# grigoriy-chirkov/primesim

Measured on AMD Instinct MI355X. Metric: simulated memory accesses/sec (uncore) at 1024 cores; % HBM roofline, higher is better.
Workload: dtype int64

## Files before the change

primesim_amd/csrc/engine.hip:

```cpp

#ifndef __HIPCC_RTC__
#include <hip/hip_runtime.h>
#include <stdint.h>
#endif

#if defined(__HIPCC_RTC__) || defined(PU_JIT_OFFLINE)
#include "primeuncore.h"
#else
#include "../../include/primeuncore.h"
#endif
#include "geometry.h"

namespace {

#ifdef PU_JIT_GEO
#include PU_JIT_GEO
#endif

template <bool LH, int NL, class T>
__device__ __forceinline__ T off_v(T c) {
#ifdef PU_JIT_GEO
    if constexpr (!LH && NL == 1) {
        uint32_t lo, hi;
        asm("s_mov_b32 %0, %1" : "=s"(lo) : "s"((uint32_t)(uint64_t)c));
// ... 665 lines not shown
        x = (int)(rem - yq * w);
        y = (int)yq;
        z = (int)zq;
    } else {
        const uint32_t yq = div_magic((uint32_t)id, c.w_magic);
        x = (int)((uint32_t)id - yq * w);
        y = (int)yq;
        z = 0;
    }
}
__device__ __forceinline__ int net_route_link(const NetCtx& c, int h, int sx, int sy, int sz, int rx, int ry, int rz,
                                              int hx, int hy) {
    const int w = c.w, w1 = c.w - 1;
    const bool e = rx > sx, n = ry > sy, u = rz > sz;
    const bool inx = h < hx, iny = h < hx + hy;
    const int hy_ = h - hx, hz_ = h - hx - hy;
    const int ax = e ? sx + h : sx - h - 1;
    const int ay = n ? sy + hy_ : sy - hy_ - 1;
    if (c.net_type != 1) return inx ? sy * w1 + ax : (w + rx) * w1 + ay;
    const int az = u ? sz + hz_ : sz - hz_ - 1;
    const int blk = w * w * w1;
    return inx ? (sz * w + sy) * w1 + ax : iny ? blk + (sz * w + rx) * w1 + ay : 2 * blk + (ry * w + rx) * w1 + az;
}


template <bool LH>
__device__ __forceinline__ void ring_dma(const NetCtx& c, int q, uint32_t head, uint32_t cnt, int slot) {
    const int ln = lane_id();
    const AS1 v2u64* R = q_ring(c, q);
    const uint32_t last = cnt - 1;
    const AS1 v2u64* ga = R + ((head + __builtin_elementwise_min((uint32_t)ln, last)) & (PU_QRING - 1));
    const AS1 v2u64* gb = R + ((head + __builtin_elementwise_min((uint32_t)ln + 64, last)) & (PU_QRING - 1));
    const uint32_t la = (uint32_t)(uintptr_t)(__attribute__((address_space(3))) v2u64*)ring_slot<LH>(slot);
    const uint32_t lo = __builtin_amdgcn_readfirstlane(la), hi = lo + 64 * sizeof(v2u64);
    unsigned keep;
    asm volatile(
        "s_waitcnt lgkmcnt(0)\n\t"
        "s_mov_b32 %0, m0\n\t"
        "s_mov_b32 m0, %3\n\t"
        "s_nop 0\n\t"
        "global_load_lds_dwordx4 %1, off\n\t"
        "s_mov_b32 m0, %4\n\t"
        "s_nop 0\n\t"
        "global_load_lds_dwordx4 %2, off\n\t"
        "s_mov_b32 m0, %0"
        : "=&s"(keep)
        : "v"(ga), "v"(gb), "s"(lo), "s"(hi)
        : "memory");
}
template <bool LH>
__device__ __forceinline__ void ring_from_lds(int slot, RingView& v) {
    const int ln = lane_id();
    const v2u64* r = ring_slot<LH>(slot);
    const v2u64 a = r[ln], b = r[ln + 64];
    v = RingView{a.x, a.y, b.x, b.y};
}

template <bool X4>
__device__ __forceinline__ void lds_dma(const AS1 char* src, uint32_t lds_base) {
    const uint32_t lo = __builtin_amdgcn_readfirstlane(lds_base);
    unsigned keep;
    if (X4)
        asm volatile("s_waitcnt lgkmcnt(0)\n\ts_mov_b32 %0, m0\n\ts_mov_b32 m0, %2\n\ts_nop 0\n\t"
                     "global_load_lds_dwordx4 %1, off\n\ts_mov_b32 m0, %0"
                     : "=&s"(keep) : "v"(src), "s"(lo) : "memory");
    else
        asm volatile("s_waitcnt lgkmcnt(0)\n\ts_mov_b32 %0, m0\n\ts_mov_b32 m0, %2\n\ts_nop 0\n\t"
                     "global_load_lds_dword %1, off\n\ts_mov_b32 m0, %0"
                     : "=&s"(keep) : "v"(src), "s"(lo) : "memory");
}
template <class T>
__device__ __forceinline__ uint32_t lds_addr(T* p) {
    return (uint32_t)(uintptr_t)(__attribute__((address_space(3))) T*)p;
}

static __shared__ v4u32 lds_dir_a[32];
static __shared__ uint32_t lds_dir_w[2][32];

#ifndef PU_PAIR_WINDOW
#define PU_PAIR_WINDOW 1
#endif
template <bool LH, bool WIDE>
constexpr bool pair_window() { return PU_PAIR_WINDOW && !LH && !WIDE; }
template <bool LH, int NL, bool WIDE>
__device__ __forceinline__ uint64_t net_transmit(const Geo* __restrict__ g, char* base_in, int src, int dst, int len,
                                                 uint64_t timer, uint32_t& hq_head, bool& pair, int len2,
                                                 int64_t base_t, int tpre) {
    constexpr bool PW = pair_window<LH, WIDE>();
    PROF_T(p_pre);
    NetCtx c;
    AS1 char* base = (AS1 char*)(char*)uni64((uint64_t)base_in);
    c.qhdr = base + OFF(g->off_qhdr);
    c.qring = base + OFF(g->off_qring);
    c.hdr_c = (uint32_t)g->nqueues * PU_HDR_AB;
    c.p0 = (uint32_t)g->header_flits;
    c.p1 = (uint32_t)g->plen_blk;
    c.router = (uint32_t)g->router_delay;
    c.link_delay = (uint32_t)g->link_delay;
    c.inject = (uint32_t)g->inject_delay;
    c.header_flits = g->header_flits;
    c.data_width = g->data_width;
    c.w = g->net_width;
    c.net_type = g->net_type;
    c.w_magic = (uint32_t)g->w_magic;
    c.w2_magic = (uint32_t)g->w2_magic;
    c.w2 = g->w2;
    c.blk_len = g->blk_len;
    c.plen_blk = g->plen_blk;
    src = (int)uni32((uint32_t)src);
    dst = (int)uni32((uint32_t)dst);
    len = (int)uni32((uint32_t)len);
    timer = uni64(timer);
    if (src == dst) {
        pair = false;
        return 0;
    }
    const int ln = lane_id();
    int plen;
    uint64_t err = 0;
    if constexpr (WIDE) {
        plen = len == 0 ? c.header_flits
             : len == c.blk_len ? c.plen_blk
             : c.header_flits + (int)ceil((double)len / (double)c.data_width);
    } else {
        plen = len == 0 ? c.header_flits : c.plen_blk;
        if (len != 0 && len != c.blk_len) err |= PU_ERRF_QUEUE;
    }
    int sx, sy, sz, rx, ry, rz;
    net_coords(c, src, sx, sy, sz);
    net_coords(c, dst, rx, ry, rz);
    const int hx = abs(rx - sx), hy = abs(ry - sy), hz = abs(rz - sz);
    const int hops = hx + hy + hz;
    bool pw = false;
    if constexpr (PW) {
        pw = pair && 2 * hops <= 64 && (hx != 0) + (hy != 0) + (hz != 0) >= 2;
        len2 = (int)uni32((uint32_t)len2);
        if (pw && len2 != 0 && len2 != c.blk_len) err |= PU_ERRF_QUEUE;
    }
    pair = pw;
    const auto plen2 = [&]() { return len2 == 0 ? c.header_flits : c.plen_blk; };
    const int thops = pw ? 2 * hops : hops;
    uint64_t t = timer + c.inject;
    uint64_t mg1 = 0;
    PROF_ADD(PF_NPRE, p_pre);
    for (int b0 = 0; b0 < thops; b0 += 64) {
        PROF_T(p_setup);
        PROF_CNT(PF_WINDOWS, 1);
        const int h = b0 + ln;
        const int nh = thops - b0 < 64 ? thops - b0 : 64;
        int rq;
        if (PW && pw) {
            const int hh = h < thops ? h : thops - 1;
            const bool bk = hh >= hops;
            rq = net_route_link(c, bk ? hh - hops : hh, bk ? rx : sx, bk ? ry : sy, bk ? rz : sz, bk ? sx : rx,
                                bk ? sy : ry, bk ? sz : rz, hx, hy);
        } else {
            rq = net_route_link(c, h < hops ? h : hops - 1, sx, sy, sz, rx, ry, rz, hx, hy);
        }
        v4u32 ha, hb, hc;
        hdr_load<LH, WIDE>(c, rq, ha, hb, hc);
        uint64_t vcache = PU_MG1_CACHE_NONE;
        if constexpr (LH) vcache = lds_qcache[rq];
        const QState hs = hdr_state<WIDE>(c, ha, hb, hc, err);
        uint32_t vhead = hs.head, vcnt = hs.count;
        uint64_t vf0 = hs.f0;
        const uint64_t vfront = vf0;
        uint64_t vd = 0;
        [[maybe_unused]] bool need = ln < nh;
        if constexpr (LH) {
            const uint64_t wmask = (1ull << PU_MG1_WAIT_BITS) - 1;
            const bool hit = need && (vcache & wmask) != wmask && hs.n < 4294967296.0 &&
                             ((uint32_t)(vcache >> PU_MG1_WAIT_BITS) ^ (uint32_t)vcache) == (uint32_t)hs.n;
            if (hit) vd = vcache & wmask;
            need = need && !hit;
            if (ballot(need)) {
                PROF_T(p_mg1);
                const uint64_t w = mg1_wait(hs);
                if (need) vd = w;
                PROF_ADD(PF_MG1RUN, p_mg1);
            }
        } else {
            PROF_T(p_mg1);
            vd = mg1_wait(hs);
            PROF_ADD(PF_MG1RUN, p_mg1);
        }
        PROF_CNT(PF_MG1LANES, (uint64_t)nh);
        PROF_CNT(PF_MG1HITS, (uint64_t)__builtin_popcountll(ballot(ln < nh && !need)));
        PROF_CNT(PF_MG1PRESENT, (uint64_t)__builtin_popcountll(ballot(ln < nh && vcache != PU_MG1_CACHE_NONE)));
        uint64_t vfin = 0;
        uint64_t X = 0;
        const int nleg = PW && pw ? 2 : 1;
#pragma clang loop unroll(disable)
        for (int leg = 0; leg < nleg; leg++) {
        const int l0 = PW && leg ? hops : 0, l1 = PW && pw ? l0 + hops : nh;
        const int pl = PW && leg ? plen2() : plen;
        const uint64_t nhm = (l1 >= 64 ? ~0ull : ((1ull << l1) - 1)) & (~0ull << l0);
        const uint64_t lb = t + (uint64_t)(ln - l0 + 1) * c.router + (uint64_t)(ln - l0) * c.link_delay;
        const uint64_t M = ballot(vfront <= lb + (uint64_t)pl) & nhm;
        uint64_t mi = M, mc = M;
        int issued = 0, consumed = 0;
        constexpr int RPF = ring_pf<LH>();
        while (mi && issued < RPF) {
            const int jj = (int)__builtin_ctzll(mi);
            mi &= mi - 1;
            ring_dma<LH>(c, (int)rl32((uint32_t)rq, jj), rl32(vhead, jj), rl32(vcnt, jj), issued % RPF);
            issued++;
        }
        PROF_ADD(PF_NSETUP, p_setup);
        PROF_T(p_hops);
        uint64_t sh = 0;
        uint64_t t0 = t;
        if (!PW || leg == 0) {
            const uint64_t e = vd + c.link_delay + c.router;
            const uint64_t S = ballot(e >= (1ull << 26)) == 0 ? (uint64_t)scan_incl_u32((uint32_t)e) : scan_incl_u64(e);
            X = S - e;
        } else {
            t0 -= rl64(X, hops);
        }
        int js = l0;
        {
            int islot = issued % RPF, cslot = 0;
            while (js < l1) {
                const uint64_t live = nhm & (~0ull << js);
                const uint64_t A = X + (t0 + c.router + sh);
                const uint64_t cand = ballot(vfront <= A + (uint64_t)pl) & live;
                const int jt = cand ? (int)__builtin_ctzll(cand) : l1;
                const uint64_t fm = jt >= 64 ? live : live & ((1ull << jt) - 1);
                vfin = selm64(fm, vfin, A + vd + (uint64_t)pl);
                mg1 += (uint64_t)(jt - js);
                if (jt == l1) {
                    t = t0 + rl64(X, l1 - 1) + rl64(vd, l1 - 1) + c.link_delay + c.router + sh;
                    break;
                }
                PROF_T(p_tree);
                PROF_CNT(PF_TREEHOPS, 1);
                PROF_T(p_pick);
                const uint64_t tj = rl64(A, jt);
                const int q = (int)rl32((uint32_t)rq, jt);
                uint32_t head = rl32(vhead, jt), cnt = rl32(vcnt, jt);
                uint64_t f0n, f1n, d;
                RingView v;
                const bool staged = mc && jt == (int)__builtin_ctzll(mc);
                int tslot = -1;
                if (staged) {
                    mc &= mc - 1;
                    PROF_T(p_wait);
                    const int newer = issued - consumed - 1;
                    static_assert(RPF <= 3, "the three-way wait covers at most 2 newer staged rings");
                    if (newer <= 0) asm volatile("s_waitcnt vmcnt(0)" ::: "memory");
                    else if (newer == 1) asm volatile("s_waitcnt vmcnt(2)" ::: "memory");
                    else asm volatile("s_waitcnt vmcnt(4)" ::: "memory");
                    PROF_ADD(PF_NWAIT, p_wait);
                    ring_from_lds<LH>(cslot, v);
                    tslot = cslot;
                    cslot = cslot == RPF - 1 ? 0 : cslot + 1;
                    consumed++;
                } else {
                    PROF_CNT(PF_DEMAND, 1);
                    ring_load(c, q, head, cnt, v);
                }
#ifdef PU_PROF
                asm volatile("s_waitcnt lgkmcnt(0)" ::: "memory");
#endif
                PROF_ADD(PF_T_LDS, p_pick);
                d = tree_op<LH>(c, q, v, head, cnt, tj, (uint64_t)pl, c.link_delay, err, f0n, f1n, tslot);
                PROF_T(p_upd);
                if (cnt >= PU_QMAX) {
                    head = (head + 1) & (PU_QRING - 1);
                    cnt--;
                    f0n = f1n;
                }
                if (staged && mi) {
                    PROF_T(p_r);
                    const int jj = (int)__builtin_ctzll(mi);
                    mi &= mi - 1;
                    ring_dma<LH>(c, (int)rl32((uint32_t)rq, jj), rl32(vhead, jj), rl32(vcnt, jj), islot);
                    islot = islot == RPF - 1 ? 0 : islot + 1;
                    issued++;
                    PROF_ADD(PF_T_REFILL, p_r);
                }
                sh += d - rl64(vd, jt);
                wl_hop(vhead, head, vcnt, cnt, vf0, f0n, vfin, tj + d + (uint64_t)pl, jt);
                t = tj + d + c.link_delay;
                js = jt + 1;
                PROF_ADD(PF_T_UPD, p_upd);
                PROF_ADD(PF_NTREE, p_tree);
            }
        }
        if (PW && pw && leg == 0) {
            t += c.router;
            t += (uint64_t)(plen - 1);
            const uint64_t dfwd = t - timer;
            const uint64_t start = (uint64_t)(base_t + (tpre + (int)dfwd));
            timer = start - dfwd;
            t = start + c.inject;
        }
        PROF_ADD(PF_NHOPS, p_hops);
        }
        PROF_T(p_wb);
        if (ln < nh) {
            QState st = hs;
            st.head = vhead;
            st.count = vcnt;
            st.f0 = vf0;
            if constexpr (WIDE) {
                st.sum_sq = st.sum_sq + (double)plen * (double)plen;
                st.sum = st.sum + (double)plen;
                st.n = st.n + 1.0;
            } else {
                st.n = st.n + 1.0;
                if ((PW && pw && ln >= hops ? plen2() : plen) != (int)c.p0) st.sum1 = st.sum1 + 1.0;
            }
            st.newest = vfin > st.newest ? vfin : st.newest;
            q_store_hdr<LH, WIDE>(c, rq, st, vhead != hs.head || vcnt != hs.count || vf0 != hs.f0);
            if constexpr (LH) lds_hq[(hq_head + (uint32_t)ln) & (PU_HQ - 1)] = (uint16_t)rq;
        }
        if constexpr (LH) {
            hq_head += (uint32_t)nh;
            asm volatile("" ::: "memory");
            if (ln == 0) *(volatile AS3 uint32_t*)&lds_hq_head = hq_head;
        }
        PROF_ADD(PF_NWB, p_wb);
    }
    PROF_T(p_post);
    t += c.router;
    t += (uint64_t)((PW && pw ? plen2() : plen) - 1);
    const uint64_t dist = (uint64_t)thops;
    {
        const uint32_t plsum = (uint32_t)(PW && pw ? plen + plen2() : plen);
        const uint64_t tot = t - timer, fl = (uint64_t)hops * (uint64_t)plsum;
        uint32_t lo = 0, hi = 0;
        lo = wlane<SN_ACC>(lo, PW && pw ? 2u : 1u);
        lo = wlane<SN_DIST>(lo, (uint32_t)dist);
        lo = wlane<SN_TOTAL>(lo, (uint32_t)tot);
        hi = wlane<SN_TOTAL>(hi, (uint32_t)(tot >> 32));
        lo = wlane<SN_PLEN>(lo, plsum);
        lo = wlane<SN_FLITS>(lo, (uint32_t)fl);
        if (WIDE || (c.p0 | c.p1) >= (1u << 23)) hi = wlane<SN_FLITS>(hi, (uint32_t)(fl >> 32));
        lo = wlane<SN_MG1>(lo, (uint32_t)mg1);
        lds_add_u64_lanes(lds_u32addr(&lds_stat[0]) + 8u * (uint32_t)ln, ((uint64_t)hi << 32) | lo, SN_NET_LANES);
    }
    if (ballot(err != 0)) err_or(PU_ERRF_QUEUE);
    PROF_ADD(PF_NPOST, p_post);
    return t - timer;
}

#ifndef PU_PF_AHEAD
#define PU_PF_AHEAD 4
#endif
static __shared__ uint32_t lds_pf_junk[64];
__device__ __forceinline__ void pf_requests(const Geo* __restrict__ g, const char* base, const pu_req* reqs,
                                            uint64_t first, uint32_t n) {
    const int ln = lane_id();
    const uint32_t j = (uint32_t)ln >> 3, k = (uint32_t)ln & 7u;
    const bool mine = j < n;
    uint64_t addr = 0;
    int core = 0;
    if (mine) {
        const pu_req q = reqs[first + j];
        addr = q.addr;
        core = q.core;
    }
    const char* p = nullptr;
    if (mine && (uint32_t)core < (uint32_t)g->num_cores) {
        const LevelGeo& L = g->lv[0];
        const uint64_t set = set_index(addr, L.offbits, L.nsets);
        const uint64_t line0 = ((uint64_t)(uint32_t)core * L.nsets + set) * L.nways;
        if (k == 0) p = (const char*)(reqs + first + j);
        else if (k <= 2) {
            if ((k - 1) * 64 < L.nways * sizeof(LineMeta)) p = base + L.off_meta + line0 * sizeof(LineMeta) + (k - 1) * 64;
        } else if (k == 3) p = base + L.off_ts + line0 * 8;
        else if (g->sys_type == 0 && k <= 6 && (k - 4) * 64 < g->dir.nways * sizeof(DirLine)) {
            const DirGeo& D = g->dir;
            int hb = (int)((addr >> g->home_offbits) & (((uint64_t)1 << g->home_mask_bits) - 1));
            if (hb >= g->N) hb &= (1 << (g->home_mask_bits - 1)) - 1;
            const uint64_t ds = set_index(addr, D.offbits, D.nsets);
            const uint64_t dl0 = ((uint64_t)(uint32_t)hb * D.csets + (ds >> D.cset_shift)) * D.nways;
            p = base + D.off_line + dl0 * sizeof(DirLine) + (k - 4) * 64;
        }
    }
    if (p) lds_dma<false>((const AS1 char*)p, lds_addr(&lds_pf_junk[0]));
}

__device__ void mg1_helper(const Geo* __restrict__ g, const char* base, const pu_req* reqs, uint64_t b, uint64_t end) {
    const bool pf_on = !g->tlb_enable;
    uint64_t pf = b;

    const int ln = lane_id();
    uint32_t tail = 0;
    for (;;) {
        const uint32_t head = uni32(*(volatile AS3 uint32_t*)&lds_hq_head);
        if (head == tail) {
            if (uni32(*(volatile AS3 uint32_t*)&lds_main_done)) {
                if (uni32(*(volatile AS3 uint32_t*)&lds_hq_head) == tail) break;
                continue;
            }
            if (pf_on) {
                const uint64_t cur = uni64(*(volatile AS3 uint64_t*)&lds_ctl.cur);
                if (cur >= b && cur < end) {
                    const uint64_t lim = end - cur > PU_PF_AHEAD ? cur + 1 + PU_PF_AHEAD : end;
                    if (pf <= cur) pf = cur + 1;
                    if (pf < lim) {
                        pf_requests(g, base, reqs, pf, (uint32_t)(lim - pf));
                        pf = lim;
                        continue;
                    }
                }
            }
            __builtin_amdgcn_s_sleep(1);
            continue;
        }
        if (head - tail > PU_HQ) tail = head - PU_HQ;
        const uint32_t n = head - tail < 64u ? head - tail : 64u;
        if ((uint32_t)ln < n) {
            const uint32_t q = lds_hq[(tail + (uint32_t)ln) & (PU_HQ - 1)];
            volatile AS3 v4u32* H = (volatile AS3 v4u32*)&lds_qhdr[(size_t)q * PU_LDS_SLOT];
            const v4u32 a = H[0];
            asm volatile("" ::: "memory");
            const v4u32 b = H[1];
            asm volatile("" ::: "memory");
            const v4u32 a2 = H[0];
            NetCtx hc;
            hc.p0 = (uint32_t)g->header_flits;
            hc.p1 = (uint32_t)g->plen_blk;
            uint64_t herr = 0;
            const QState st = hdr_state<false>(hc, a, b, v4u32{0u, 0u, 0u, 0u}, herr);
            const uint64_t w = mg1_wait(st);
            const uint64_t wmask = (1ull << PU_MG1_WAIT_BITS) - 1;
            const bool same = a.x == a2.x && a.y == a2.y && a.z == a2.z && a.w == a2.w;
            const bool st_ok = same && !herr && w < wmask && st.n < 4294967296.0;
            if (st_ok)
                *(volatile AS3 uint64_t*)&lds_qcache[q] = w | ((uint64_t)((uint32_t)st.n ^ (uint32_t)w) << PU_MG1_WAIT_BITS);
#ifdef PU_PROF
            const uint64_t nst = __builtin_popcountll(ballot(st_ok));
            if (ln == 0) atomicAdd(&lds_prof[PF_MG1STORED], (unsigned long long)nst);
#endif
        }
        PROF_CNT(PF_MG1BATCH, 1);
        tail += n;
    }
}

template <int NL, bool LH = false, bool WIDE = false>
struct Engine {
    const Geo* __restrict__ g;
    char* base;
    int ln;

    int dly;
    bool hit;
    uint32_t hq_head;

    __device__ __forceinline__ void init_shared(int32_t pool_top, uint64_t page_next, uint64_t last_addr) const {
        lds_eng.pool_top = pool_top;
        lds_eng.stop = 0;
        lds_eng.page_next = page_next;
        lds_eng.last_addr = last_addr;
    }


    template <class T>
    __device__ __forceinline__ T* at(uint64_t off) const {
        return reinterpret_cast<T*>(base + off);
    }

    __device__ __forceinline__ NetCtx net_ctx() const {
        NetCtx c;
        c.qhdr = (AS1 char*)base + OFF(g->off_qhdr);
        c.qring = (AS1 char*)base + OFF(g->off_qring);
        c.hdr_c = (uint32_t)g->nqueues * PU_HDR_AB;
        c.p0 = c.p1 = (uint32_t)g->bus_latency;
        c.router = (uint32_t)g->router_delay;
        c.link_delay = (uint32_t)g->link_delay;
        c.inject = (uint32_t)g->inject_delay;
        c.header_flits = g->header_flits;
        c.data_width = g->data_width;
        c.w = g->net_width;
        c.net_type = g->net_type;
        return c;
    }
    __device__ __forceinline__ uint64_t transmit(int src, int dst, int len, uint64_t timer) {
        PROF_T(p0);
        bool pair = false;
        uint64_t d = net_transmit<LH, NL, WIDE>(g, base, src, dst, len, timer, hq_head, pair, 0, 0, 0);
        PROF_ADD(PF_NET, p0);
        return d;
    }
    __device__ __forceinline__ uint64_t transmit_leg(int src, int dst, int len, uint64_t timer, bool& pair, int len2,
                                                     int64_t base_t, int tpre) {
        PROF_T(p0);
        uint64_t d = net_transmit<LH, NL, WIDE>(g, base, src, dst, len, timer, hq_head, pair, len2, base_t, tpre);
        PROF_ADD(PF_NET, p0);
        return d;
    }

    __device__ __forceinline__ void set_load(SetView& v, const LineMeta* meta, const int64_t* ts,
                                             uint64_t nsets, uint64_t nways, int offbits, int idxbits,
                                             uint64_t cache_index, uint64_t addr) const {
        v.set = set_index(addr, offbits, nsets);
        v.tag = addr >> (offbits + idxbits);
        v.line0 = (uint64_t)(((uint32_t)cache_index * (uint32_t)nsets + (uint32_t)v.set) * (uint32_t)nways);
        set_chunk(v, meta, ts, nways, 0);
    }
    __device__ __forceinline__ void set_chunk(SetView& v, const LineMeta* meta, const int64_t* ts, uint64_t nways,
                                              uint32_t w0) const {
        v.w0 = w0;
        const uint64_t w = (uint64_t)w0 + (uint64_t)ln;
        if (w < nways) {
            LineMeta m = meta[v.line0 + w];
            v.mtag = m.tag;
            v.mid = m.id;
            v.mst = m.state;
            v.mts = ts[v.line0 + w];
        } else {
            v.mtag = 0;
            v.mid = 0;
            v.mst = ST_I;
            v.mts = INT64_MAX;
        }
    }
    static __device__ __forceinline__ bool wide(uint64_t nways) { return nways > 64; }
    static __device__ __forceinline__ int wl(const SetView& v, int way) { return way - (int)v.w0; }
    __device__ __forceinline__ int set_find(SetView& v, const LineMeta* meta, const int64_t* ts, uint64_t nways,
                                            int prog) const {
        if (!wide(nways)) {
            uint64_t m = ballot((uint64_t)ln < nways && v.mst != ST_I && v.mid == prog && v.mtag == v.tag);
            return m ? (int)__builtin_ctzll(m) : -1;
        }
        for (uint32_t c = 0;; c += 64) {
            if (c != v.w0) set_chunk(v, meta, ts, nways, c);
            const uint64_t m =
                ballot((uint64_t)c + (uint64_t)ln < nways && v.mst != ST_I && v.mid == prog && v.mtag == v.tag);
            if (m) return (int)c + (int)__builtin_ctzll(m);
            if ((uint64_t)c + 64 >= nways) return -1;
        }
    }
    __device__ __forceinline__ int set_replace(SetView& v, LineMeta* meta, const int64_t* ts, uint64_t nways,
                                               int offbits, int idxbits, int prog, uint32_t* old_state,
                                               uint64_t* old_addr, int* old_prog) const {
        int way = -1;
        bool invalid = false;
        if (!wide(nways)) {
            const uint64_t inv = ballot((uint64_t)ln < nways && v.mst == ST_I);
            if (inv) {
                invalid = true;
                way = (int)__builtin_ctzll(inv);
            } else {
                way = lru_way(v.mts, (uint64_t)ln < nways ? lane_here(ln) : 64, nways);
            }
        } else {
            int64_t best = INT64_MAX;
            for (uint32_t c = 0; (uint64_t)c < nways && !invalid; c += 64) {
                if (c != v.w0) set_chunk(v, meta, ts, nways, c);
                const bool mine = (uint64_t)c + (uint64_t)ln < nways;
                const uint64_t inv = ballot(mine && v.mst == ST_I);
                if (inv) {
                    invalid = true;
                    way = (int)c + (int)__builtin_ctzll(inv);
                } else {
                    const int lw = lru_way(v.mts, mine ? ln : 64, 64);
                    const int64_t t = (int64_t)rl64((uint64_t)v.mts, lw);
                    if (way < 0 || t < best) {
                        best = t;
                        way = (int)c + lw;
                    }
                }
            }
            if ((uint32_t)way - v.w0 >= 64u) set_chunk(v, meta, ts, nways, (uint32_t)way & ~63u);
        }
        const int wlane = wl(v, way);
        if (invalid) {
            *old_state = ST_I;
            *old_addr = 0;
            *old_prog = 0;
        } else {
            *old_state = rl32(v.mst, wlane);
            *old_addr = (v.set << offbits) | (rl64(v.mtag, wlane) << (offbits + idxbits));
            *old_prog = (int)rl32((uint32_t)v.mid, wlane);
        }
        if (ln == wlane) {
            v.mtag = v.tag;
            v.mid = prog;
            meta[v.line0 + (uint64_t)way] = LineMeta{v.tag, prog, v.mst};
        }
        return way;
    }
    __device__ __forceinline__ void set_state(SetView& v, LineMeta* meta, int way, uint32_t st) const {
        if (ln == wl(v, way)) {
            v.mst = st;
            meta[v.line0 + (uint64_t)way].state = st;
        }
    }
    __device__ __forceinline__ void set_ts(SetView& v, int64_t* ts, int way, int64_t t) const {
        if (ln == wl(v, way)) {
            v.mts = t;
            ts[v.line0 + (uint64_t)way] = t;
        }
    }

    __device__ __forceinline__ void mark_alive(int l, int cid) const {
        for (int k = l; k < NL; k++) {
            if constexpr (kAliveLds) {
                const uint32_t bit = (uint32_t)(alive_base(k) + cid), m = 1u << (bit & 31);
                const uint32_t w = uni32(lds_alive[bit >> 5]);
                if (!(w & m)) {
                    if (ln == (cid & 63)) at<uint32_t>(OFF(g->lv[k].off_alive))[cid] = 1u;
                    if (ln == 0) lds_alive[bit >> 5] = w | m;
                }
            } else {
                if (ln == (cid & 63)) at<uint32_t>(OFF(g->lv[k].off_alive))[cid] = 1u;
            }
            if (k + 1 < NL) cid = cid * g->lv[k].share / g->lv[k + 1].share;
        }
    }
    template <int K>
    __device__ __forceinline__ void count(uint64_t off_cnt, int cid, int which) const {
        if constexpr (kCntSum) stat_add(SN_CNT0 + 4 * K + which, 1);
        else gatomic_add_u64_lane0(at<uint64_t>(off_cnt) + (size_t)cid * 4 + which, 1ull);
    }

    __device__ __forceinline__ int dram(uint64_t addr, int64_t t) {
        stat_add(SN_DRAM, 1);
        if (g->dram_banks == 0) return g->dram_access_time;
        const uint64_t row = uni64(addr) >> g->dram_row_shift;
        const uint64_t bank = row & (uint64_t)(g->dram_banks - 1);
        const uint64_t page = (row >> g->dram_bank_shift) + 1;
        t = (int64_t)uni64((uint64_t)t);
        DramBank* B = at<DramBank>(OFF(g->off_dram)) + bank;
        const int64_t ready = (int64_t)uni64((uint64_t)B->ready);
        const uint64_t open = uni64(B->open);
        const int64_t start = ready > t ? ready : t;
// ... 161 lines not shown
        sh = idx;
    }

    enum ProbeMode { PR_NONE, PR_ONE, PR_INLINE, PR_POOL, PR_ALL };
    __device__ __forceinline__ int probe(int mode, int one, uint32_t nsh, uint64_t sh, bool inval, int reply_len, int home,
                         const Req& r, int64_t timer, int delay) {
        constexpr int last = NL - 1;
        const bool single = mode == PR_ONE;
        const int64_t base_t = single ? timer : timer + delay;
        int pipe = single ? delay : 0, mx = 0;
        int pbase = 0;
        uint64_t rem = mode == PR_POOL ? pool_word(sh) : 0ull;
        uint32_t k = 0;
        while (true) {
            int p;
            if (mode == PR_ONE) {
                if (k) break;
                p = one;
            } else if (mode == PR_INLINE) {
                if (k >= nsh) break;
                p = (int)((sh >> (16 * k)) & 0xFFFF);
            } else if (mode == PR_POOL) {
                uint64_t m = ballot(rem != 0);
                while (!m && pbase + 64 < g->dir.nwords) {
                    pbase += 64;
                    rem = pool_word(sh, pbase);
                    m = ballot(rem != 0);
                }
                if (!m) break;
                const int w = (int)__builtin_ctzll(m);
                p = (pbase + w) * 64 + (int)__builtin_ctzll(rl64(rem, w));
                if (ln == w) rem &= rem - 1;
            } else if (mode == PR_ALL) {
                if ((int)k >= g->num_cores) break;
                p = (int)k;
            } else {
                break;
            }
            k++;
            int t = pipe;
            if constexpr (pair_window<LH, WIDE>()) {
                const uint64_t start = (uint64_t)(base_t + t);
                t += inval ? down<last, true>(p, r) : down<last, false>(p, r);
#pragma clang loop unroll(disable)
                for (int back = 0; back < 2; back++) {
                    bool paired = !back;
                    t += (int)transmit_leg(back ? p : home, back ? home : p, back ? reply_len : 0,
                                           back ? (uint64_t)(base_t + t) : start, paired, reply_len, base_t, t);
                    if (paired) break;
                }
            } else {
#pragma clang loop unroll(disable)
                for (int back = 0; back < 2; back++) {
                    t += (int)transmit(back ? p : home, back ? home : p, back ? reply_len : 0, (uint64_t)(base_t + t));
                    if (!back) t += inval ? down<last, true>(p, r) : down<last, false>(p, r);
                }
            }
            if (single) return t;
            mx = t > mx ? t : mx;
            pipe += g->header_flits;
        }
        return delay + mx;
    }

    __device__ __forceinline__ int dir_stage(int home, uint64_t addr, bool no_hops) const {
        const DirGeo& D = g->dir;
        if (D.nways > 32) return 0;
        const uint64_t set = set_index(addr, D.offbits, D.nsets);
        const uint64_t line0 = (uint64_t)(((uint32_t)home * (uint32_t)D.csets + (uint32_t)(set >> D.cset_shift)) * (uint32_t)D.nways);
        if ((uint64_t)ln < D.nways) {
            const AS1 char* lp = (const AS1 char*)(const char*)(at<DirLine>(OFF(D.off_line)) + line0 + (uint64_t)ln);
            lds_dma<true>(lp, lds_addr(&lds_dir_a[0]));
            lds_dma<false>(lp + 16, lds_addr(&lds_dir_w[0][0]));
            lds_dma<false>(lp + 20, lds_addr(&lds_dir_w[1][0]));
        }
        return no_hops ? 2 : 1;
    }
    __device__ __forceinline__ int access_home(int cid, int home, const Req& r, int64_t timer, uint32_t* out_state, int staged = 0) {
        PROF_T(p0);
        int d = access_home_impl(cid, home, r, timer, out_state, staged);
        PROF_ADD(PF_HOME, p0);
        return d;
    }
    __device__ __forceinline__ int access_home_impl(int cid, int home, const Req& r, int64_t timer, uint32_t* out_state,
                                    int staged) {
        PROF_T(p_ld);
        const DirGeo& D = g->dir;
        const bool shared = g->shared_llc != 0;
        constexpr int last = NL - 1;
        const int blk = (int)g->lv[last].block;
        DirLine* lines = at<DirLine>(OFF(D.off_line));
        if (!kCntSum && ln == (home & 63)) at<uint32_t>(OFF(D.off_alive))[home] = 1u;
        const uint64_t set = set_index(r.addr, D.offbits, D.nsets);
        const uint64_t tag = r.addr >> (D.offbits + D.idxbits);
        const uint64_t line0 = (uint64_t)(((uint32_t)home * (uint32_t)D.csets + (uint32_t)(set >> D.cset_shift)) * (uint32_t)D.nways);
        bool mine = (uint64_t)ln < D.nways;
        uint32_t dw0 = 0;
        DirLine m;
        if (staged == 1) {
            if constexpr (LH) asm volatile("s_waitcnt vmcnt(0)" ::: "memory");
            else asm volatile("s_waitcnt vmcnt(8)" ::: "memory");
        } else if (staged == 2) {
            asm volatile("s_waitcnt vmcnt(0)" ::: "memory");
        }
        if (mine && staged) {
            const v4u32 a = lds_dir_a[ln];
            m.tag = u64of(a.x, a.y);
            m.ts = (int64_t)u64of(a.z, a.w);
            const int lw = lane_here(ln);
            m.w = u64of(lds_dir_w[0][lw], lds_dir_w[1][lw]);
        } else if (mine) {
            m = lines[line0 + (uint64_t)ln];
        } else {
            m.tag = 0; m.ts = INT64_MAX; m.w = 0;
        }
        uint32_t m_state = dir_state(m.w);
        const uint32_t want10 = prog10(r.prog), m_p10 = (uint32_t)(m.w >> 54);
        int32_t* side = at<int32_t>(OFF(D.off_prog));
        int32_t m_prog = (int32_t)m_p10;
        if (want10 == PU_DIR_PROG_ESC || ballot(mine && m_p10 == PU_DIR_PROG_ESC)) {
            if (mine && m_p10 == PU_DIR_PROG_ESC) m_prog = side[line0 + (uint64_t)ln];
        }
        auto dir_chunk = [&](uint32_t c) {
            dw0 = c;
            mine = (uint64_t)c + (uint64_t)ln < D.nways;
            if (mine) {
                m = lines[line0 + (uint64_t)c + (uint64_t)ln];
            } else {
                m.tag = 0; m.ts = INT64_MAX; m.w = 0;
            }
            m_state = dir_state(m.w);
            const uint32_t p10 = (uint32_t)(m.w >> 54);
            m_prog = (int32_t)p10;
            if (mine && p10 == PU_DIR_PROG_ESC) m_prog = side[line0 + (uint64_t)c + (uint64_t)ln];
        };
        uint64_t hm = ballot(mine && m_state != ST_I && m_prog == r.prog && m.tag == tag);
        int way = hm ? (int)__builtin_ctzll(hm) : -1;
        if (wide(D.nways) && !hm) {
            for (uint32_t c = 64; (uint64_t)c < D.nways; c += 64) {
                dir_chunk(c);
                hm = ballot(mine && m_state != ST_I && m_prog == r.prog && m.tag == tag);
                if (hm) {
                    way = (int)c + (int)__builtin_ctzll(hm);
                    break;
                }
            }
        }
        PROF_ADD(PF_HOME_LD, p_ld);
        count<PU_CNT_DIR>(OFF(D.off_cnt), home, 0);
        int delay = D.access_time;
        uint32_t st, nsh;
        uint64_t sh;
        int pmode = PR_NONE, pone = 0, preply = 0;
        bool pinval = true;
        uint32_t psh_n = 0;
        uint64_t psh = 0;
        Req pr = r;
        int extra_dram = 0;
        bool release_set = false, miss_fill = false;
        if (way < 0 && r.type != PU_WB) {
            uint32_t old_st = ST_I;
            uint64_t old_addr = 0;
            int old_prog = 0;
            bool inv = false;
            if (!wide(D.nways)) {
                const uint64_t im = ballot(mine && m_state == ST_I);
                inv = im != 0;
                if (inv) {
                    way = (int)__builtin_ctzll(im);
                } else {
                    way = lru_way(m.ts, mine ? ln : 64, D.nways);
                }
            } else {
                int64_t best = INT64_MAX;
                for (uint32_t c = 0; (uint64_t)c < D.nways && !inv; c += 64) {
                    if (c != dw0) dir_chunk(c);
                    const uint64_t im = ballot(mine && m_state == ST_I);
                    if (im) {
                        inv = true;
                        way = (int)c + (int)__builtin_ctzll(im);
                    } else {
                        const int lw = lru_way(m.ts, mine ? ln : 64, 64);
                        const int64_t t = (int64_t)rl64((uint64_t)m.ts, lw);
                        if (way < 0 || t < best) {
                            best = t;
                            way = (int)c + lw;
                        }
                    }
                }
                if ((uint32_t)way - dw0 >= 64u) dir_chunk((uint32_t)way & ~63u);
            }
            const int wlane = way - (int)dw0;
            const uint64_t ww = rl64(m.w, wlane);
            if (!inv) {
                old_st = dir_state(ww);
                old_addr = (set << D.offbits) | (rl64(m.tag, wlane) << (D.offbits + D.idxbits));
                old_prog = (int)rl32((uint32_t)m_prog, wlane);
            }
            dir_sharers(ww, nsh, sh);
            if (old_st != ST_I) {
                count<PU_CNT_DIR>(OFF(D.off_cnt), home, 2);
                pr = Req{old_addr, old_prog, PU_RD};
                if (old_st == ST_M || old_st == ST_E) {
                    pmode = PR_ONE;
                    pone = first_sharer(nsh, sh);
                    preply = (!shared || old_st == ST_M) ? blk : 0;
                    extra_dram = 1;
                } else if (old_st == ST_S) {
                    pmode = nsh == PU_SH_POOL ? PR_POOL : PR_INLINE;
                } else if (old_st == ST_B) {
                    pmode = PR_ALL;
                }
            }
            st = r.type == PU_WR ? ST_M : ST_E;
            count<PU_CNT_DIR>(OFF(D.off_cnt), home, 1);
            release_set = true;
            miss_fill = true;
        } else if (way < 0) {
            err_or(PU_ERRF_WB_MISS);
            *out_state = ST_I;
            return delay;
        } else {
            const uint64_t ww = rl64(m.w, way - (int)dw0);
            st = dir_state(ww);
            dir_sharers(ww, nsh, sh);
            if (r.type == PU_WR) {
                if (st == ST_M || st == ST_E) {
                    pmode = PR_ONE;
                    pone = first_sharer(nsh, sh);
                    preply = blk;
                } else if (st == ST_S) {
                    pmode = nsh == PU_SH_POOL ? PR_POOL : PR_INLINE;
                    if (!shared) extra_dram = 2;
                } else if (st == ST_B) {
                    pmode = PR_ALL;
                    if (!shared) extra_dram = 2;
                }
                st = ST_M;
                release_set = true;
            } else if (r.type == PU_RD) {
                if (st == ST_M || st == ST_E) {
                    pmode = PR_ONE;
                    pone = first_sharer(nsh, sh);
                    preply = blk;
                    pinval = false;
                    st = ST_S;
                } else if (st == ST_S) {
                    if (!shared) delay += dram(r.addr, timer + delay);
                    if (g->protocol_type == 1 && count_sharers(nsh, sh) >= g->max_num_sharers) st = ST_B;
                } else if (st == ST_B) {
                    if (!shared) delay += dram(r.addr, timer + delay);
                } else if (st == ST_V) {
                    st = ST_E;
                }
            } else {
                st = shared ? ST_V : ST_I;
                pool_release(nsh, sh);
                nsh = 0;
                sh = 0;
                dram(r.addr, timer + delay);
            }
        }
        if (pmode != PR_NONE) {
            if (pmode == PR_ALL) stat_add(SN_BCAST, 1);
            psh_n = nsh;
            psh = sh;
            delay = probe(pmode, pone, psh_n, psh, pinval, preply, home, pr, timer, delay);
        }
        if (extra_dram == 1) dram(pr.addr, timer + delay);
        if (extra_dram == 2) delay += dram(r.addr, timer + delay);
        if (release_set) {
            pool_release(nsh, sh);
            nsh = 1;
            sh = (uint64_t)cid;
            if (miss_fill) delay += dram(r.addr, timer + delay);

        } else if (r.type == PU_RD) {
            add_sharer(nsh, sh, cid);
        }
        *out_state = st == ST_B ? ST_S : st;
        if (ln == way - (int)dw0) {
            lines[line0 + (uint64_t)way] = DirLine{tag, timer, dir_word(nsh, sh, st, want10)};
            if (want10 == PU_DIR_PROG_ESC) side[line0 + (uint64_t)way] = r.prog;
        }
        return delay;
    }

    __device__ __forceinline__ int home_of(uint64_t addr) const {
        int hb = (int)((addr >> g->home_offbits) & (((uint64_t)1 << g->home_mask_bits) - 1));
        if (hb < g->N) return hb;
        return hb & ((1 << (g->home_mask_bits - 1)) - 1);
    }

    template <int LV>
    __device__ __forceinline__ uint32_t mesi(int cid, const Req& r, int64_t timer) {
        const LevelGeo& L = g->lv[LV];
        constexpr bool kLast = LV == NL - 1;
        LineMeta* meta = at<LineMeta>(OFF(L.off_meta));
        int64_t* tsa = at<int64_t>(OFF(L.off_ts));
        SetView v;
        PROF_T(p_set);
        set_load(v, meta, tsa, L.nsets, L.nways, L.offbits, L.idxbits, (uint64_t)cid, r.addr);
        mark_alive(LV, cid);
        if (L.has_bus) {
            stat_add(SN_BUSACC, 1);
            uint64_t bl = (uint64_t)g->bus_latency, mg1 = 0, err = 0;
            int db = (int)q_op<LH, WIDE>(net_ctx(), L.bus_q0 + cid, (uint64_t)(timer + dly), bl, bl, mg1, err);
            stat_add(SN_MG1, mg1);
            if (err) err_or(err);
            stat_add(SN_BUSCONT, (uint64_t)(int64_t)db);
            dly += db;
        }
        if (!hit) count<LV>(OFF(L.off_cnt), cid, 0);
        dly += L.access_time;
        int way = set_find(v, meta, tsa, L.nways, r.prog);
        PROF_ADD(LV == 0 ? PF_SETL0 : PF_SETLN, p_set);
        bool is_miss = false, call_parent = false;
        int64_t ptimer = 0;
        uint32_t ret = ST_M;
        bool tx_wb = false, tx_req = false;
        int wb_home = 0, req_reply = 0;
        Req wb_req = r;
        if (way >= 0) {
            set_ts(v, tsa, way, timer + dly);
            hit = true;
            const uint32_t st = rl32(v.mst, wl(v, way));
            if (r.type == PU_WR) {
                if constexpr (!kLast) {
                    if (st != ST_M) {
                        set_state(v, meta, way, ST_I);
                        call_parent = true;
                        ptimer = timer + dly;
                    }
                } else {
                    if (st == ST_S) {
                        tx_req = true;
                        req_reply = 0;
                    }
                }
                ret = ST_M;
            } else {
                if (st != ST_S) dly += children<LV, false>(cid, r);
                return ST_S;
            }
        } else {
            is_miss = true;
            uint32_t old_st;
            uint64_t old_addr;
            int old_prog;
            way = set_replace(v, meta, tsa, L.nways, L.offbits, L.idxbits, r.prog, &old_st, &old_addr, &old_prog);
            if (old_st != ST_I) {
                count<LV>(OFF(L.off_cnt), cid, 2);
                Req o{old_addr, old_prog, PU_RD};
                dly += children<LV, true>(cid, o);
                if (old_st == ST_M || old_st == ST_E) {
                    count<LV>(OFF(L.off_cnt), cid, 3);
                    if constexpr (kLast) {
                        tx_wb = true;
                        wb_home = home_of(old_addr);
                        wb_req = Req{old_addr, old_prog, PU_WB};
                    }
                }
            }
            set_ts(v, tsa, way, timer + dly);
            if constexpr (!kLast) {
                call_parent = true;
                ptimer = timer;
            } else {
                tx_req = true;
                req_reply = (int)L.block;
            }
        }
        if constexpr (!kLast) {
            if (call_parent) {
                const int parent = cid * L.share / g->lv[LV + 1].share;
                const uint32_t ns = mesi<LV + 1>(parent, r, ptimer);
                set_state(v, meta, way, ns);
                if (is_miss) ret = ns;
            }
        } else {
            const int req_home = home_of(r.addr);
            int leg = tx_wb ? 0 : (tx_req ? 1 : 3);
            while (leg < 3) {
                const bool wb = leg == 0;
                const int home = wb ? wb_home : req_home;
                const int src = leg == 2 ? home : cid, dst = leg == 2 ? cid : home;
                const int len = wb ? (int)L.block : (leg == 1 ? 0 : req_reply);
                const int staged = leg == 1 ? dir_stage(home, r.addr, src == dst) : 0;
                const int d1 = (int)transmit(src, dst, len, (uint64_t)(timer + dly));
                if (!wb) dly += d1;
                if (leg == 2) break;
                uint32_t hs;
                const int d2 = access_home(cid, home, wb ? wb_req : r, timer + dly, &hs, staged);
                if (!wb) {
                    dly += d2;
                    if (is_miss) ret = hs;
                }
                leg = wb ? (tx_req ? 1 : 3) : 2;
            }
            set_state(v, meta, way, is_miss ? ret : ST_M);
        }
        if (is_miss) count<LV>(OFF(L.off_cnt), cid, 1);
        return ret;
    }

    __device__ __forceinline__ bool snoop(int cid, const Req& r, int mode) {
        constexpr int last = NL - 1;
        const LevelGeo& L = g->lv[last];
        LineMeta* meta = at<LineMeta>(OFF(L.off_meta));
        const uint64_t set = set_index(r.addr, L.offbits, L.nsets);
        const uint64_t tag = r.addr >> (L.offbits + L.idxbits);
        bool any = false;
        for (int base = 0; base < L.ncaches; base += 64) {
            const int c = base + ln;
            int myway = -1;
            uint32_t myst = ST_I;
            if (c < L.ncaches && c != cid) {
                const LineMeta* sp = meta + ((uint64_t)c * L.nsets + set) * L.nways;
                for (uint64_t w = L.nways; w-- > 0;) {
                    const LineMeta m = sp[w];
                    if (m.state != ST_I && m.id == r.prog && m.tag == tag) {
                        myway = (int)w;
                        myst = m.state;
                    }
                }
            }
            uint64_t hits = ballot(myway >= 0);
            while (hits) {
                const int k = (int)__builtin_ctzll(hits);
                hits &= hits - 1;
                const int i = base + k;
                const int way = (int)rl32((uint32_t)myway, k);
                const uint32_t st = rl32(myst, k);
                any = true;
                if (mode == 2) children<last, false>(i, r);
                else children<last, true>(i, r);
                if (ln == 0) meta[((uint64_t)i * L.nsets + set) * L.nways + (uint64_t)way].state = mode == 2 ? ST_S : ST_I;
                if (mode != 0 && (st == ST_M || st == ST_E)) return any;
            }
        }
        return any;
    }

    template <int LV>
    __device__ __forceinline__ uint32_t mesi_bus(int cid, const Req& r, int64_t timer) {
        const LevelGeo& L = g->lv[LV];
        constexpr bool kLast = LV == NL - 1;
        LineMeta* meta = at<LineMeta>(OFF(L.off_meta));
        int64_t* tsa = at<int64_t>(OFF(L.off_ts));
        SetView v;
        set_load(v, meta, tsa, L.nsets, L.nways, L.offbits, L.idxbits, (uint64_t)cid, r.addr);
        mark_alive(LV, cid);
        if (L.has_bus) {
            stat_add(SN_BUSACC, 1);
            uint64_t bl = (uint64_t)g->bus_latency, mg1 = 0, err = 0;
            int db = (int)q_op<LH, WIDE>(net_ctx(), L.bus_q0 + cid, (uint64_t)(timer + dly), bl, bl, mg1, err);
            stat_add(SN_MG1, mg1);
            if (err) err_or(err);
            stat_add(SN_BUSCONT, (uint64_t)(int64_t)db);
            dly += db;
        }
        dly += L.access_time;
        if (!hit) count<LV>(OFF(L.off_cnt), cid, 0);
        int way = set_find(v, meta, tsa, L.nways, r.prog);
        bool is_miss = false, call_parent = false;
// ... 764 lines not shown
```

Before: 350.4 million.

## Chain request, probe and reply network legs into shared hop windows

Splits the home directory access into a decide phase and a rest phase so the last-level miss path can batch consecutive network legs (request to home, then reply to requester or forward to a single sharer) into one wavefront hop window with distinct second destinations. It also stages the directory set early in the last-level mesi call and adds an opaque register barrier for LRU lane selection. The aim is fewer separate net_transmit windows and serialized queue passes per miss. The cost is more complex control flow and register pressure, plus a risk of timing-model divergence when paths share links.

```diff
diff --git a/primesim_amd/csrc/engine.hip b/primesim_amd/csrc/engine.hip
--- a/primesim_amd/csrc/engine.hip
+++ b/primesim_amd/csrc/engine.hip
@@ -771,11 +771,20 @@
 #endif
 template <bool LH, bool WIDE>
 constexpr bool pair_window() { return PU_PAIR_WINDOW && !LH && !WIDE; }
+#ifndef PU_CHAIN_WINDOW
+#define PU_CHAIN_WINDOW 1
+#endif
+#ifndef PU_CHAIN_STAGE_EARLY
+#define PU_CHAIN_STAGE_EARLY 1
+#endif
+template <bool LH, bool WIDE>
+constexpr bool chain_window() { return PU_CHAIN_WINDOW && pair_window<LH, WIDE>(); }
 template <bool LH, int NL, bool WIDE>
 __device__ __forceinline__ uint64_t net_transmit(const Geo* __restrict__ g, char* base_in, int src, int dst, int len,
                                                  uint64_t timer, uint32_t& hq_head, bool& pair, int len2,
-                                                 int64_t base_t, int tpre) {
+                                                 int64_t base_t, int tpre, int dst2, int post, uint64_t& dfirst) {
     constexpr bool PW = pair_window<LH, WIDE>();
+    constexpr bool CW = chain_window<LH, WIDE>();
     PROF_T(p_pre);
     NetCtx c;
     AS1 char* base = (AS1 char*)(char*)uni64((uint64_t)base_in);
@@ -800,6 +809,7 @@
     dst = (int)uni32((uint32_t)dst);
     len = (int)uni32((uint32_t)len);
     timer = uni64(timer);
+    dfirst = 0;
     if (src == dst) {
         pair = false;
         return 0;
@@ -821,14 +831,31 @@
     const int hx = abs(rx - sx), hy = abs(ry - sy), hz = abs(rz - sz);
     const int hops = hx + hy + hz;
     bool pw = false;
-    if constexpr (PW) {
+    int cx = sx, cy = sy, cz = sz, hx2 = hx, hy2 = hy, hops2 = hops;
+    if constexpr (CW) {
+        if (pair) {
+            dst2 = (int)uni32((uint32_t)dst2);
+            tpre = (int)uni32((uint32_t)tpre);
+            post = (int)uni32((uint32_t)post);
+            net_coords(c, dst2, cx, cy, cz);
+            hx2 = abs(cx - rx);
+            hy2 = abs(cy - ry);
+            hops2 = hx2 + hy2 + abs(cz - rz);
+            const bool share = (sy == ry && sz == rz && (sx - rx) * (cx - rx) > 0) ||
+                               (rx == cx && sz == rz && (sy - ry) * (cy - ry) > 0) ||
+                               (rx == cx && ry == cy && (sz - rz) * (cz - rz) > 0);
+            pw = hops2 != 0 && hops + hops2 <= 64 && !share;
+        }
+        len2 = (int)uni32((uint32_t)len2);
+        if (pw && len2 != 0 && len2 != c.blk_len) err |= PU_ERRF_QUEUE;
+    } else if constexpr (PW) {
         pw = pair && 2 * hops <= 64 && (hx != 0) + (hy != 0) + (hz != 0) >= 2;
         len2 = (int)uni32((uint32_t)len2);
         if (pw && len2 != 0 && len2 != c.blk_len) err |= PU_ERRF_QUEUE;
     }
     pair = pw;
     const auto plen2 = [&]() { return len2 == 0 ? c.header_flits : c.plen_blk; };
-    const int thops = pw ? 2 * hops : hops;
+    const int thops = pw ? hops + hops2 : hops;
     uint64_t t = timer + c.inject;
     uint64_t mg1 = 0;
     PROF_ADD(PF_NPRE, p_pre);
@@ -841,8 +868,8 @@
         if (PW && pw) {
             const int hh = h < thops ? h : thops - 1;
             const bool bk = hh >= hops;
-            rq = net_route_link(c, bk ? hh - hops : hh, bk ? rx : sx, bk ? ry : sy, bk ? rz : sz, bk ? sx : rx,
-                                bk ? sy : ry, bk ? sz : rz, hx, hy);
+            rq = net_route_link(c, bk ? hh - hops : hh, bk ? rx : sx, bk ? ry : sy, bk ? rz : sz, bk ? cx : rx,
+                                bk ? cy : ry, bk ? cz : rz, bk ? hx2 : hx, bk ? hy2 : hy);
         } else {
             rq = net_route_link(c, h < hops ? h : hops - 1, sx, sy, sz, rx, ry, rz, hx, hy);
         }
@@ -881,7 +908,7 @@
         const int nleg = PW && pw ? 2 : 1;
 #pragma clang loop unroll(disable)
         for (int leg = 0; leg < nleg; leg++) {
-        const int l0 = PW && leg ? hops : 0, l1 = PW && pw ? l0 + hops : nh;
+        const int l0 = PW && leg ? hops : 0, l1 = PW && pw ? l0 + (leg ? hops2 : hops) : nh;
         const int pl = PW && leg ? plen2() : plen;
         const uint64_t nhm = (l1 >= 64 ? ~0ull : ((1ull << l1) - 1)) & (~0ull << l0);
         const uint64_t lb = t + (uint64_t)(ln - l0 + 1) * c.router + (uint64_t)(ln - l0) * c.link_delay;
@@ -980,7 +1007,8 @@
             t += c.router;
             t += (uint64_t)(plen - 1);
             const uint64_t dfwd = t - timer;
-            const uint64_t start = (uint64_t)(base_t + (tpre + (int)dfwd));
+            dfirst = dfwd;
+            const uint64_t start = (uint64_t)(base_t + (tpre + (int)dfwd) + (CW ? post : 0));
             timer = start - dfwd;
             t = start + c.inject;
         }
@@ -1017,7 +1045,9 @@
     const uint64_t dist = (uint64_t)thops;
     {
         const uint32_t plsum = (uint32_t)(PW && pw ? plen + plen2() : plen);
-        const uint64_t tot = t - timer, fl = (uint64_t)hops * (uint64_t)plsum;
+        const uint64_t tot = t - timer;
+        const uint64_t fl = CW && pw ? (uint64_t)hops * (uint64_t)plen + (uint64_t)hops2 * (uint64_t)plen2()
+                                     : (uint64_t)hops * (uint64_t)plsum;
         uint32_t lo = 0, hi = 0;
         lo = wlane<SN_ACC>(lo, PW && pw ? 2u : 1u);
         lo = wlane<SN_DIST>(lo, (uint32_t)dist);
@@ -1031,6 +1061,7 @@
     }
     if (ballot(err != 0)) err_or(PU_ERRF_QUEUE);
     PROF_ADD(PF_NPOST, p_post);
+    if (!(PW && pw)) dfirst = t - timer;
     return t - timer;
 }
 
@@ -1171,18 +1202,33 @@
     __device__ __forceinline__ uint64_t transmit(int src, int dst, int len, uint64_t timer) {
         PROF_T(p0);
         bool pair = false;
-        uint64_t d = net_transmit<LH, NL, WIDE>(g, base, src, dst, len, timer, hq_head, pair, 0, 0, 0);
+        uint64_t dfirst;
+        uint64_t d = net_transmit<LH, NL, WIDE>(g, base, src, dst, len, timer, hq_head, pair, 0, 0, 0, 0, 0, dfirst);
+        PROF_ADD(PF_NET, p0);
+        return d;
+    }
+    __device__ __forceinline__ uint64_t transmit_chain(int src, int dst, int len, uint64_t timer, bool& pair, int dst2,
+                                                       int len2, int64_t base_t, int tpre, int post, uint64_t& dfirst) {
+        PROF_T(p0);
+        uint64_t d = net_transmit<LH, NL, WIDE>(g, base, src, dst, len, timer, hq_head, pair, len2, base_t, tpre, dst2, post,
+                                                dfirst);
         PROF_ADD(PF_NET, p0);
         return d;
     }
     __device__ __forceinline__ uint64_t transmit_leg(int src, int dst, int len, uint64_t timer, bool& pair, int len2,
                                                      int64_t base_t, int tpre) {
         PROF_T(p0);
-        uint64_t d = net_transmit<LH, NL, WIDE>(g, base, src, dst, len, timer, hq_head, pair, len2, base_t, tpre);
+        uint64_t dfirst;
+        uint64_t d = net_transmit<LH, NL, WIDE>(g, base, src, dst, len, timer, hq_head, pair, len2, base_t, tpre, src, 0,
+                                                dfirst);
         PROF_ADD(PF_NET, p0);
         return d;
     }
 
+    __device__ __forceinline__ int lru_lane(bool mine, int w) const {
+        if constexpr (chain_window<LH, WIDE>()) asm volatile("" : "+v"(w));
+        return mine ? w : 64;
+    }
     __device__ __forceinline__ void set_load(SetView& v, const LineMeta* meta, const int64_t* ts,
                                              uint64_t nsets, uint64_t nways, int offbits, int idxbits,
                                              uint64_t cache_index, uint64_t addr) const {
@@ -1235,7 +1281,7 @@
                 invalid = true;
                 way = (int)__builtin_ctzll(inv);
             } else {
-                way = lru_way(v.mts, (uint64_t)ln < nways ? lane_here(ln) : 64, nways);
+                way = lru_way(v.mts, lru_lane((uint64_t)ln < nways, lane_here(ln)), nways);
             }
         } else {
             int64_t best = INT64_MAX;
@@ -1563,8 +1609,30 @@
         PROF_ADD(PF_HOME, p0);
         return d;
     }
+    struct HomeDec {
+        int way;
+        uint32_t dw0, st, nsh;
+        uint64_t sh;
+        int pmode, pone, preply;
+        bool pinval;
+        Req pr;
+        int pre_dram;
+        int extra_dram;
+        bool release_set, miss_fill, wb_miss;
+    };
+    __device__ __forceinline__ int home_after(const HomeDec& h) const {
+        int d = 0;
+        if (h.pre_dram == 1) d += g->dram_access_time;
+        if (h.extra_dram == 2) d += g->dram_access_time;
+        if (h.release_set && h.miss_fill) d += g->dram_access_time;
+        return d;
+    }
     __device__ __forceinline__ int access_home_impl(int cid, int home, const Req& r, int64_t timer, uint32_t* out_state,
                                     int staged) {
+        const HomeDec h = home_decide(home, r, staged);
+        return home_rest(h, cid, home, r, timer, false, 0, out_state);
+    }
+    __device__ __forceinline__ HomeDec home_decide(int home, const Req& r, int staged) {
         PROF_T(p_ld);
         const DirGeo& D = g->dir;
         const bool shared = g->shared_llc != 0;
@@ -1629,15 +1697,12 @@
         }
         PROF_ADD(PF_HOME_LD, p_ld);
         count<PU_CNT_DIR>(OFF(D.off_cnt), home, 0);
-        int delay = D.access_time;
         uint32_t st, nsh;
         uint64_t sh;
         int pmode = PR_NONE, pone = 0, preply = 0;
         bool pinval = true;
-        uint32_t psh_n = 0;
-        uint64_t psh = 0;
         Req pr = r;
-        int extra_dram = 0;
+        int pre_dram = 0, extra_dram = 0;
         bool release_set = false, miss_fill = false;
         if (way < 0 && r.type != PU_WB) {
             uint32_t old_st = ST_I;
@@ -1650,7 +1715,7 @@
                 if (inv) {
                     way = (int)__builtin_ctzll(im);
                 } else {
-                    way = lru_way(m.ts, mine ? ln : 64, D.nways);
+                    way = lru_way(m.ts, lru_lane(mine, ln), D.nways);
                 }
             } else {
                 int64_t best = INT64_MAX;
@@ -1699,8 +1764,11 @@
             miss_fill = true;
         } else if (way < 0) {
             err_or(PU_ERRF_WB_MISS);
-            *out_state = ST_I;
-            return delay;
+            HomeDec h{};
+            h.way = -1;
+            h.pr = r;
+            h.wb_miss = true;
+            return h;
         } else {
             const uint64_t ww = rl64(m.w, way - (int)dw0);
             st = dir_state(ww);
@@ -1727,42 +1795,78 @@
                     pinval = false;
                     st = ST_S;
                 } else if (st == ST_S) {
-                    if (!shared) delay += dram(r.addr, timer + delay);
+                    if (!shared) pre_dram = 1;
                     if (g->protocol_type == 1 && count_sharers(nsh, sh) >= g->max_num_sharers) st = ST_B;
                 } else if (st == ST_B) {
-                    if (!shared) delay += dram(r.addr, timer + delay);
+                    if (!shared) pre_dram = 1;
                 } else if (st == ST_V) {
                     st = ST_E;
                 }
             } else {
                 st = shared ? ST_V : ST_I;
-                pool_release(nsh, sh);
-                nsh = 0;
-                sh = 0;
-                dram(r.addr, timer + delay);
-            }
-        }
-        if (pmode != PR_NONE) {
-            if (pmode == PR_ALL) stat_add(SN_BCAST, 1);
-            psh_n = nsh;
-            psh = sh;
-            delay = probe(pmode, pone, psh_n, psh, pinval, preply, home, pr, timer, delay);
-        }
-        if (extra_dram == 1) dram(pr.addr, timer + delay);
-        if (extra_dram == 2) delay += dram(r.addr, timer + delay);
-        if (release_set) {
+                pre_dram = 2;
+            }
+        }
+        HomeDec h;
+        h.way = way;
+        h.dw0 = dw0;
+        h.st = st;
+        h.nsh = nsh;
+        h.sh = uni64(sh);
+        h.pmode = pmode;
+        h.pone = (int)uni32((uint32_t)pone);
+        h.preply = preply;
+        h.pinval = pinval;
+        h.pr = Req{uni64(pr.addr), (int)uni32((uint32_t)pr.prog), (int)uni32((uint32_t)pr.type)};
+        h.pre_dram = pre_dram;
+        h.extra_dram = extra_dram;
+        h.release_set = release_set;
+        h.miss_fill = miss_fill;
+        h.wb_miss = false;
+        return h;
+    }
+    __device__ __forceinline__ int home_rest(const HomeDec& h, int cid, int home, const Req& r, int64_t timer, bool probed,
+                                             int pdelay, uint32_t* out_state) {
+        const DirGeo& D = g->dir;
+        int delay = D.access_time;
+        if (h.wb_miss) {
+            *out_state = ST_I;
+            return delay;
+        }
+        uint32_t st = h.st, nsh = h.nsh;
+        uint64_t sh = h.sh;
+        if (r.type == PU_WB) {
+            pool_release(nsh, sh);
+            nsh = 0;
+            sh = 0;
+        }
+        if (h.pre_dram == 1) delay += dram(r.addr, timer + delay);
+        if (h.pre_dram == 2) dram(r.addr, timer + delay);
+        if (probed) {
+            delay = pdelay;
+        } else if (h.pmode != PR_NONE) {
+            if (h.pmode == PR_ALL) stat_add(SN_BCAST, 1);
+            delay = probe(h.pmode, h.pone, nsh, sh, h.pinval, h.preply, home, h.pr, timer, delay);
+        }
+        if (h.extra_dram == 1) dram(h.pr.addr, timer + delay);
+        if (h.extra_dram == 2) delay += dram(r.addr, timer + delay);
+        if (h.release_set) {
             pool_release(nsh, sh);
             nsh = 1;
             sh = (uint64_t)cid;
-            if (miss_fill) delay += dram(r.addr, timer + delay);
+            if (h.miss_fill) delay += dram(r.addr, timer + delay);
 
         } else if (r.type == PU_RD) {
             add_sharer(nsh, sh, cid);
         }
         *out_state = st == ST_B ? ST_S : st;
-        if (ln == way - (int)dw0) {
-            lines[line0 + (uint64_t)way] = DirLine{tag, timer, dir_word(nsh, sh, st, want10)};
-            if (want10 == PU_DIR_PROG_ESC) side[line0 + (uint64_t)way] = r.prog;
+        if (ln == h.way - (int)h.dw0) {
+            const uint64_t set = set_index(r.addr, D.offbits, D.nsets);
+            const uint64_t tag = r.addr >> (D.offbits + D.idxbits);
+            const uint64_t line0 = (uint64_t)(((uint32_t)home * (uint32_t)D.csets + (uint32_t)(set >> D.cset_shift)) * (uint32_t)D.nways);
+            const uint32_t want10 = prog10(r.prog);
+            at<DirLine>(OFF(D.off_line))[line0 + (uint64_t)h.way] = DirLine{tag, timer, dir_word(nsh, sh, st, want10)};
+            if (want10 == PU_DIR_PROG_ESC) at<int32_t>(OFF(D.off_prog))[line0 + (uint64_t)h.way] = r.prog;
         }
         return delay;
     }
@@ -1782,6 +1886,7 @@
         SetView v;
         PROF_T(p_set);
         set_load(v, meta, tsa, L.nsets, L.nways, L.offbits, L.idxbits, (uint64_t)cid, r.addr);
+        if constexpr (kLast && chain_window<LH, WIDE>() && PU_CHAIN_STAGE_EARLY) dir_stage(home_of(r.addr), r.addr, true);
         mark_alive(LV, cid);
         if (L.has_bus) {
             stat_add(SN_BUSACC, 1);
@@ -1862,6 +1967,89 @@
         } else {
             const int req_home = home_of(r.addr);
             int leg = tx_wb ? 0 : (tx_req ? 1 : 3);
+            if constexpr (chain_window<LH, WIDE>()) {
+                const DirGeo& D = g->dir;
+                const bool fixed = g->dram_banks == 0;
+                way = (int)uni32((uint32_t)way);
+                const int64_t tm = (int64_t)uni64((uint64_t)timer);
+                int dl = (int)uni32((uint32_t)dly);
+                HomeDec hd{};
+                bool probing = false;
+                int pt = 0;
+                while (leg < 3) {
+                    const bool wb = leg == 0;
+                    const int home = wb ? wb_home : req_home;
+                    int src = leg == 2 ? home : cid, dst = leg == 2 ? cid : home;
+                    int len = wb ? (int)L.block : (leg == 1 ? 0 : req_reply);
+                    uint64_t start = (uint64_t)(tm + dl);
+                    bool pair = false;
+                    int dst2 = 0, len2 = 0, tpre = 0, post = 0;
+                    if (probing) {
+                        src = hd.pone;
+                        len = hd.preply;
+                        start = (uint64_t)(tm + dl + pt);
+                        pair = true;
+                        dst2 = cid;
+                        len2 = req_reply;
+                        tpre = dl + pt + home_after(hd);
+                    } else if (leg < 2) {
+                        int staged = 0;
+                        if (leg == 1)
+                            staged = tx_wb || !PU_CHAIN_STAGE_EARLY ? dir_stage(home, r.addr, true) : (D.nways > 32 ? 0 : 2);
+                        hd = home_decide(home, wb ? wb_req : r, staged);
+                        if (leg == 1 && fixed && hd.pmode == PR_NONE) {
+                            pair = true;
+                            dst2 = cid;
+                            len2 = req_reply;
+                            tpre = dl + D.access_time + home_after(hd);
+                        } else if (leg == 1 && fixed && hd.pmode == PR_ONE) {
+                            pair = true;
+                            dst2 = hd.pone;
+                            tpre = dl;
+                            post = D.access_time;
+                        }
+                    }
+                    uint64_t dfirst;
+                    const int dsum = (int)uni32((uint32_t)transmit_chain(src, dst, len, start, pair, dst2, len2, tm, tpre,
+                                                                         post, dfirst));
+                    const int dfst = (int)uni32((uint32_t)dfirst);
+                    if (leg == 2) {
+                        dl += dsum;
+                        break;
+                    }
+                    const bool probed = probing;
+                    if (probed) {
+                        pt += dfst;
+                    } else {
+                        if (!wb) dl += dfst;
+                        if (leg == 1 && pair && hd.pmode == PR_ONE) {
+                            pt = D.access_time + (dsum - dfst);
+                            pt += hd.pinval ? down<NL - 1, true>(hd.pone, hd.pr) : down<NL - 1, false>(hd.pone, hd.pr);
+                            pt = (int)uni32((uint32_t)pt);
+                            probing = true;
+                            continue;
+                        }
+                    }
+                    probing = false;
+                    uint32_t hs;
+                    const HomeDec hnow = hd;
+                    hd = HomeDec{};
+                    const int d2 = home_rest(hnow, cid, home, wb ? wb_req : r, tm + dl, probed, pt, &hs);
+                    pt = 0;
+                    if (wb) {
+                        leg = tx_req ? 1 : 3;
+                        continue;
+                    }
+                    dl += d2;
+                    if (is_miss) ret = hs;
+                    if (pair) {
+                        dl += (dsum - dfst);
+                        break;
+                    }
+                    leg = 2;
+                }
+                dly = dl;
+            } else
             while (leg < 3) {
                 const bool wb = leg == 0;
                 const int home = wb ? wb_home : req_home;
```

After: 327.1 million. -6.7%, worse.
